# WilliamLewww/lens_trace

Hardware: AMD Instinct MI355X
Metric: Mrays/s (primary+secondary+shadow), 1M-tri @4K (higher is better)
Workload: dtype f32

## Files before the change

### include/lenstrace_hip.h

```cpp
#ifndef LENSTRACE_HIP_H
#define LENSTRACE_HIP_H

#include <stddef.h>
#include <stdint.h>

#ifdef __cplusplus
extern "C" {
#endif

#define LT_HIP_ABI_VERSION 4

typedef struct lt_hip_context lt_hip_context;

enum {
  LT_OK = 0,
  LT_ERR_INVALID_ARGUMENT = 1,
  LT_ERR_NO_DEVICE = 2,
  LT_ERR_HIP = 3,
  LT_ERR_NO_SCENE = 4,
  LT_ERR_BAD_SCENE = 5,
  LT_ERR_BUFFER_TOO_SMALL = 6,
  LT_ERR_UNKNOWN_PROGRAM = 7
};

// ... 301 lines not shown

int lt_hip_entry_cut_chunk_counts(lt_hip_context* ctx, uint64_t* out23);

int lt_hip_read_entry_cuts(lt_hip_context* ctx, void* out, uint64_t capacity, uint64_t* out_bytes);

int lt_hip_entry_cut_pruned_test_host(const uint32_t* refs, const uint16_t* parents, const uint16_t* kids, const uint8_t* survives, uint32_t n,
                                      uint32_t cap, uint32_t* out, uint32_t* count);

int lt_hip_entry_cut_chunks_test_host(const int32_t* heights, const uint32_t* chunks, const uint32_t* entries, const uint32_t* which, uint64_t n,
                                      uint32_t* out);

int lt_hip_entry_cut_triangle_test_host(const float* origins, const float* light_boxes, const float* triangles, uint64_t n, uint8_t* out);

int lt_hip_clear_item_counts(lt_hip_context* ctx, uint64_t* out5);

int lt_hip_clear_items_test_host(const uint32_t* marks, const uint32_t* order, uint32_t n, uint32_t groups, uint32_t tile_w, uint32_t tile_h,
                                 uint32_t tiles_in_call, uint32_t* table, uint8_t* map);

#ifdef __cplusplus
}
#endif
#endif
```

### lens_trace_amd/_capi.py

```python
import ctypes
import os

_HERE = os.path.dirname(os.path.abspath(__file__))
LIB_PATH = os.environ.get("LT_HIP_LIBRARY") or os.path.join(_HERE, "lib", "liblenstrace-hip.so")

(LT_OK, LT_ERR_INVALID_ARGUMENT, LT_ERR_NO_DEVICE, LT_ERR_HIP, LT_ERR_NO_SCENE, LT_ERR_BAD_SCENE,
 LT_ERR_BUFFER_TOO_SMALL, LT_ERR_UNKNOWN_PROGRAM) = range(8)
STATUS_NAMES = ["LT_OK", "LT_ERR_INVALID_ARGUMENT", "LT_ERR_NO_DEVICE", "LT_ERR_HIP", "LT_ERR_NO_SCENE",
                "LT_ERR_BAD_SCENE", "LT_ERR_BUFFER_TOO_SMALL", "LT_ERR_UNKNOWN_PROGRAM"]

PROGRAM_BASIC, PROGRAM_BASIC_LIGHTING, PROGRAM_ACCUMULATOR, PROGRAM_GLOBAL_ILLUMINATION, PROGRAM_GLOBAL_ILLUMINATION_25 = range(5)
PROGRAM_CUSTOM_OPENCL = 5
KERNEL_MODE_LINEAR, KERNEL_MODE_TILE = 0, 1
RENDER_FLAG_STATS = 1
RENDER_FLAG_PIXEL_COUNTERS = 2
RENDER_FLAG_DEVICE_LIBM = 4
RENDER_FLAG_PORTABLE_MATH = 8
RENDER_FLAG_STRICT_MATH = 16
RENDER_FLAG_NO_WALK_TIMING = 32
TRACE_CLOSEST, TRACE_ANY = 0, 1
TRACE_FLAG_COHERENT = 0x100
TRACE_FIRST_K, TRACE_COUNT = 0, 1
TRACE_MAX_HITS = 8
TRACE_LIST_FLAG_FILL_ONLY = 0x200
# ... 11 lines not shown
           "lt_hip_synchronize", "lt_hip_get_stats", "lt_hip_own_hierarchy", "lt_hip_own_wide", "lt_hip_read_scene_structure",
           "lt_hip_trace_rays", "lt_hip_trace_rays_device", "lt_hip_trace_hits", "lt_hip_trace_hits_device",
           "lt_hip_trace_hits_list", "lt_hip_trace_hits_list_device",
           "lt_hip_shade_rays", "lt_hip_shade_rays_device", "lt_hip_shade_paths", "lt_hip_shade_paths_device",
           "lt_hip_trace_surface", "lt_hip_trace_surface_device", "lt_hip_surface_at", "lt_hip_surface_at_device",
           "lt_hip_nearest_points", "lt_hip_nearest_points_device", "lt_hip_nearest_points_host",
           "lt_hip_nearest_k", "lt_hip_nearest_k_device", "lt_hip_nearest_k_host",
           "lt_hip_nearest_list", "lt_hip_nearest_list_device", "lt_hip_nearest_list_host",
           "lt_hip_overlap_boxes", "lt_hip_overlap_boxes_device", "lt_hip_overlap_boxes_host",
           "lt_hip_overlap_tris", "lt_hip_overlap_tris_device", "lt_hip_overlap_tris_host",
           "lt_hip_overlap_boxes_list", "lt_hip_overlap_boxes_list_device", "lt_hip_overlap_boxes_list_host",
           "lt_hip_overlap_tris_list", "lt_hip_overlap_tris_list_device", "lt_hip_overlap_tris_list_host",
           "lt_hip_entry_cut_counts", "lt_hip_entry_cut_test_host",
           "lt_hip_entry_cut_leaf_counts", "lt_hip_entry_cut_triangle_test_host",
           "lt_hip_entry_cut_chunk_counts", "lt_hip_entry_cut_chunks_test_host", "lt_hip_read_entry_cuts",
           "lt_hip_entry_cut_pruned_test_host", "lt_hip_clear_item_counts", "lt_hip_clear_items_test_host"]


class RenderDesc(ctypes.Structure):
    _fields_ = [("struct_size", ctypes.c_uint32), ("program", ctypes.c_int32), ("kernel_mode", ctypes.c_int32),
                ("width", ctypes.c_uint32), ("height", ctypes.c_uint32), ("depth", ctypes.c_uint32),
                ("camera", ctypes.c_uint8 * 28),
                ("frame_first", ctypes.c_uint32), ("frame_count", ctypes.c_uint32), ("accumulate", ctypes.c_uint32),
                ("accumulate_base", ctypes.c_uint32),
                ("tile_w", ctypes.c_uint32), ("tile_h", ctypes.c_uint32), ("tile_first", ctypes.c_uint32),
                ("tile_stride", ctypes.c_uint32),
                ("gi_max_depth", ctypes.c_int32), ("flags", ctypes.c_uint32)]


class Stats(ctypes.Structure):
    _fields_ = [("rays", ctypes.c_uint64), ("shadow_rays", ctypes.c_uint64), ("node_visits", ctypes.c_uint64),
# ... 244 lines not shown
        L.lt_hip_entry_cut_chunk_counts.argtypes = [vp, ctypes.POINTER(u64)]
        L.lt_hip_entry_cut_chunk_counts.restype = i32
        L.lt_hip_entry_cut_chunks_test_host.argtypes = [vp, vp, vp, vp, u64, vp]
        L.lt_hip_entry_cut_chunks_test_host.restype = i32
    if hasattr(L, "lt_hip_read_entry_cuts"):
        L.lt_hip_read_entry_cuts.argtypes = [vp, vp, u64, ctypes.POINTER(u64)]
        L.lt_hip_read_entry_cuts.restype = i32
    if hasattr(L, "lt_hip_entry_cut_pruned_test_host"):
        L.lt_hip_entry_cut_pruned_test_host.argtypes = [vp, vp, vp, vp, ctypes.c_uint32, ctypes.c_uint32, vp, vp]
        L.lt_hip_entry_cut_pruned_test_host.restype = i32
    if hasattr(L, "lt_hip_clear_item_counts"):
        L.lt_hip_clear_item_counts.argtypes = [vp, ctypes.POINTER(u64)]
        L.lt_hip_clear_item_counts.restype = i32
        L.lt_hip_clear_items_test_host.argtypes = [vp, vp] + [ctypes.c_uint32] * 5 + [vp, vp]
        L.lt_hip_clear_items_test_host.restype = i32
    for name in EXPORTS:
        if not hasattr(L, name) and os.environ.get("LT_HIP_LIBRARY"):
            continue
        if name not in ("lt_hip_last_error",):
            getattr(L, name).restype = i32
    if L.lt_hip_abi_version() != 4:
        raise ImportError("liblenstrace-hip.so ABI version mismatch")
    _lib = L
    return L


def program_from_path(path):
    out = ctypes.c_int(0)
    rc = load().lt_hip_program_from_path(path.encode(), ctypes.byref(out))
    if rc:
# ... 36 lines not shown
```

### lens_trace_amd/csrc/lt_capi.hip

```cpp
#include "lt_kernel.hpp"
#include "lt_retree.hpp"
#include "lt_own16.hpp"
#include "lt_prep.hpp"
#include "lt_query.hpp"
#include "lt_nearest.hpp"
#include "lt_overlap.hpp"
#include "lt_tritri.hpp"
#include "lt_overlist.hpp"
#include "lt_shade.hpp"
#include "lt_paths.hpp"

#include "../../include/lenstrace_hip.h"

#include <dlfcn.h>

#include <sched.h>

#include <algorithm>
#include <atomic>
#include <chrono>
#include <exception>
#include <thread>
#include <type_traits>
#include <cmath>
// ... 311 lines not shown
  bool cuts_valid = false;
  unsigned long long* d_cut_stats = nullptr;
  uint32_t cuts_leaves = 0;
  uint32_t cuts_chunks = 0;
  uint32_t cuts_node_chunks = 0;
  uint32_t cuts_plane_squares = 0;
  uint64_t cut_builds = 0;
  uint32_t* d_items = nullptr;
  uint64_t items_words = 0;
  uint32_t* d_foldmap = nullptr;
  uint64_t foldmap_words = 0;
  uint32_t items_groups = 0;
  bool items_folds = false;
  unsigned long long* d_item_stats = nullptr;
  uint64_t item_builds = 0;
  bool last_folded = false;
  bool last_tabled = false;
  unsigned long long* h_item_stats = nullptr;
  hipEvent_t items_ev = nullptr;
  int items_worth = -1;
  uint64_t scene_generation = 0;
  hipEvent_t render_ev = nullptr;
  hipStream_t render_stream = nullptr;
  bool render_ev_recorded = false;
  uint64_t d_samples_bytes = 0;
  uint32_t* d_order = nullptr;
  uint64_t order_capacity = 0;
  std::vector<uint32_t> order_key;
  uint32_t order_head[8] = {0};
  int cu_count = 256;
// ... 726 lines not shown
  bool fused_frames = !env_off("LT_FUSED_FRAMES");
  uint64_t fused_bytes = 16ull << 30;
  uint32_t debug_lds_rows = 0;
  bool debug_calibration = getenv("LT_DEBUG_CALIBRATION") != nullptr;
  bool debug_camera_hits = getenv("LT_DEBUG_CAMERA_HITS") != nullptr;
  bool pinned_readback = !env_off("LT_PINNED_READBACK");
  bool camera_hits = !env_off("LT_CAMERA_HITS");
  bool camera_hits_keep = !env_off("LT_CAMERA_HITS_KEEP");
  bool entry_cut = !env_off("LT_ENTRY_CUT");
  uint32_t entry_cut_leaves = 512;
  uint32_t entry_cut_chunks = (uint32_t)lt_entry_cut::kDefaultChunks;
  uint32_t entry_cut_node_chunks = (uint32_t)lt_entry_cut::kDefaultNodeChunks;
  bool clear_items = !env_off("LT_CLEAR_ITEMS");
  bool clear_items_fold = true;
  bool clear_items_force = false;
  uint32_t shadow_frames = 2;
  bool debug_shadow_frames = getenv("LT_DEBUG_SHADOW_FRAMES") != nullptr;
  RenderKnobs() {
    if (const char* e = getenv("LT_SHADOW_PACKETS")) shadow_packets = std::max(0, std::min(3, atoi(e)));
    if (const char* e = getenv("LT_SHADOW_SPREAD")) shadow_spread = (float)atof(e);
    if (const char* e = getenv("LT_GI_MEGAKERNEL")) gi_wavefront = atoi(e) == 0;
    if (const char* e = getenv("LT_TRACE_REFILL")) trace_refill = (uint32_t)std::max(1, std::min(64, atoi(e)));
    if (const char* e = getenv("LT_FUSED_BYTES")) fused_bytes = strtoull(e, nullptr, 10);
    if (const char* e = getenv("LT_DEBUG_LDS_ROWS")) debug_lds_rows = (uint32_t)std::max(1, std::min(160, atoi(e)));
    if (const char* e = getenv("LT_ENTRY_CUT_LEAVES")) {
      const int v = atoi(e);
      entry_cut_leaves = v <= 0 ? 0u : v == 1 ? 512u : (uint32_t)std::min(v, 1 << 20);
    }
    if (const char* e = getenv("LT_ENTRY_CUT_CHUNKS")) entry_cut_chunks = (uint32_t)std::max(1, std::min(lt_entry_cut::kMaxChunks, atoi(e)));
    if (const char* e = getenv("LT_ENTRY_CUT_NODE_CHUNKS")) entry_cut_node_chunks = (uint32_t)std::max(1, std::min(lt_entry_cut::kMaxChunks, atoi(e)));
// ... 670 lines not shown
                            hipStream_t s, const RenderKnobs& k, ReadBack* rb) {
  if (const int rc = check_render_desc(ctx, d, p, out_device, out_bytes)) return rc;
  LT_HIP_CHECK(ctx, hipSetDevice(ctx->device));
  const bool stats = (d->flags & (LT_RENDER_FLAG_STATS | LT_RENDER_FLAG_PIXEL_COUNTERS)) != 0;
  const int devlibm = (d->flags & LT_RENDER_FLAG_PORTABLE_MATH) ? 0 : (d->flags & LT_RENDER_FLAG_STRICT_MATH) ? 1 : 2;
  SceneDev sc = scene_dev(ctx, k, devlibm);
  FrameParams fp = frame_params(d, p, k);
  uint32_t camFrame;
  memcpy(&camFrame, d->camera + 24, 4);
  const uint32_t frames = d->frame_count ? d->frame_count : 1;
  const uint64_t nblocks = p.squares();

  if (!ctx->render_ev) LT_HIP_CHECK(ctx, hipEventCreateWithFlags(&ctx->render_ev, hipEventDisableTiming));
  if (ctx->render_ev_recorded && s != ctx->render_stream) LT_HIP_CHECK(ctx, hipStreamWaitEvent(s, ctx->render_ev, 0));
  if (stats) LT_HIP_CHECK(ctx, hipMemsetAsync(ctx->d_stats, 0, 8 * sizeof(unsigned long long), s));
  if (k.persistent) {
    const uint64_t queueBytes = ((uint64_t)frames + 1) * 8 * kQueueStride * sizeof(uint32_t);
    LT_HIP_CHECK(ctx, grow_scratch(ctx, ctx->d_queues, ctx->queue_frames, (uint64_t)frames + 1, queueBytes));
    LT_HIP_CHECK(ctx, hipMemsetAsync(ctx->d_queues, 0, queueBytes, s));
    if (k.square_order)
      if (const int rc = ensure_square_order(ctx, d, p, fp.sinYaw == 0.0f, s, &fp.order, fp.orderHead)) return rc;
  }
  FusionPlan fu;
  if (const int rc = plan_fusion(ctx, k, d, p, frames, stats, fp.giMaxDepth, fu)) return rc;
  const bool fused = fu.chunk > 1, meanInLaunch = d->frame_count && d->accumulate && !fused;
  const uint32_t firstFrames = fused ? std::min(fu.chunk, frames) : 1u;
  const std::vector<uint32_t> shadowKey = {(uint32_t)d->program, d->width, d->height, p.tileW, p.tileH, p.tileFirst, p.tileStride,
                                           firstFrames == 1u ? 1u : firstFrames < 8u ? 2u : 8u};
  const bool queueOk = d->program == LT_PROGRAM_ACCUMULATOR && k.persistent && !stats && ctx->d_rank8 != nullptr && !meanInLaunch &&
                       nblocks * firstFrames * kBlock + (uint64_t)ctx->cu_count * 2048u <= 0xffffffffull;
// ... 40 lines not shown
      float* outPtr = out;
      void* args[] = {(void*)&sc, (void*)&fp, (void*)&outPtr, (void*)&statsPtr, (void*)&queues};
      const hipFunction_t fn = devlibm == 2 ? up.lds : devlibm == 1 ? up.ldsStrict : up.ldsPortable;
      LT_HIP_CHECK(ctx, hipModuleLaunchKernel(fn, grid.x, 1, 1, kBlock, 1, 1, lds, s, args, nullptr));
    } else {
      FrameParams fl = fp;
      const uint32_t groups = (nf + 1u) / 2u;
      if (k.clear_items && k.persistent && !stats && d->program == LT_PROGRAM_ACCUMULATOR && (shadowMode == 1 || shadowMode == 2) && fp.entryCuts != nullptr && ctx->cuts_valid && fp.cameraHits != nullptr &&
          std::all_of(fp.orderHead, fp.orderHead + 8, [](uint32_t h) { return h == 0u; }) && std::min(shadowGroup, k.shadow_frames) >= 2u &&
          nf >= 2u && fp.squareMajor != 0u && nblocks * groups < 0x80000000ull) {
        const bool fold = k.clear_items_fold && fused && mean_in_quads(fp.depth, paddedTiles, out_device) && p.tileW % 8u == 0u;
        if (const int rc = ensure_clear_items(ctx, call, fl, groups, fold, p.floats, out_device, (int32_t)(d->accumulate_base + f))) return rc;
      }
      foldMap = (const unsigned char*)fl.foldMap;
      tabled = fl.itemTable != nullptr;
      if (shadowMode < 0 && calibrate)
        if (const int rc = calibrate_shadow_walk(ctx, call, sc, fp, grid, out, queues, queueOk, shadowKey, shadowMode, shadowGroup)) return rc;
      if (const int rc = launch_walk(ctx, call, sc, (uint32_t)std::max(0, shadowMode), shadowGroup, fl, grid, out, queues)) return rc;
    }
    LT_HIP_CHECK(ctx, hipGetLastError());
    call.launches++;
    if (fp.storeHeadHits) {
      ctx->camhits_key.swap(hitsKey);
      fp.storeHeadHits = 0u;
    }
    if (fused)
      if (const int rc = launch_running_mean(ctx, s, fp, p.floats, nf, (int32_t)(d->accumulate_base + f), paddedTiles, out_device, f + nf >= frames ? rb : nullptr, foldMap))
        return rc;
    ctx->last_folded = (launchIndex != 0 && ctx->last_folded) || foldMap != nullptr;
    ctx->last_tabled = (launchIndex != 0 && ctx->last_tabled) || tabled;
// ... 1524 lines not shown
  out4[0] = out4[1] = out4[2] = 0;
  out5[4] = ctx->last_tabled ? 1 : 0;
  out4[3] = ctx->item_builds;
  if (ctx->cuts_valid && ctx->items_groups != 0u && ctx->d_item_stats) {
    LT_HIP_CHECK(ctx, hipSetDevice(ctx->device));
    if (ctx->render_ev_recorded) LT_HIP_CHECK(ctx, hipEventSynchronize(ctx->render_ev));
    unsigned long long h[2];
    LT_HIP_CHECK(ctx, hipMemcpy(h, ctx->d_item_stats, sizeof(h), hipMemcpyDeviceToHost));
    out4[0] = h[0];
    out4[1] = h[1];
    out4[2] = ctx->last_folded ? h[1] : 0;
  }
  return LT_OK;
}

extern "C" int lt_hip_clear_items_test_host(const uint32_t* marks, const uint32_t* order, uint32_t n, uint32_t groups, uint32_t tile_w, uint32_t tile_h,
                                            uint32_t tiles_in_call, uint32_t* table, uint8_t* map) {
  if (!marks || !table || groups == 0 || (uint64_t)n * groups >= 0x80000000ull) return LT_ERR_INVALID_ARGUMENT;
  const uint32_t bptx = (tile_w + 7u) / 8u, bpty = (tile_h + 7u) / 8u;
  if (map && (tile_w == 0 || tile_w % 8u != 0 || tile_h == 0 || (uint64_t)tiles_in_call * bptx * bpty != n)) return LT_ERR_INVALID_ARGUMENT;
  for (uint32_t xcd = 0; xcd < 8u; xcd++) {
    const uint32_t share = xcd_share_size(n, xcd), start = xcd_share_start(n, xcd);
    uint32_t* const dst = table + lt_entry_cut::kItemHeader + (size_t)start * groups;
    uint32_t at = 0;
    for (uint32_t local = 0; local < share; local++) {
      const uint32_t word0 = marks[start + local];
      lt_entry_cut::item_write(dst + at, word0, local, groups);
      at += lt_entry_cut::item_entries(word0, groups);
      if (map) {
        const uint32_t b = order ? order[start + local] : start + local;
// ... 36 lines not shown
```

### lens_trace_amd/csrc/lt_device.hpp

```cpp
#pragma once
#ifndef __HIPCC_RTC__
#include <hip/hip_runtime.h>
#include <stdint.h>
#else
typedef unsigned char uint8_t;
typedef unsigned short uint16_t;
typedef unsigned int uint32_t;
typedef int int32_t;
typedef unsigned long long uint64_t;
#endif

#ifndef M_PI
#define M_PI 3.14159265358979323846
#endif

#include "lt_walk_asm.hpp"

namespace lt {

constexpr int kBlock = 64;
constexpr int kLdsStack = 32;
constexpr int kQueueStride = 64;
constexpr int kPacketEntry = 4;
constexpr int kPacketRows = 2;
constexpr int kMaxStack = 64;
constexpr int kOwnRows = 16;
constexpr int kOwnDeep = 48;
constexpr int kTraceRows = 10;
constexpr int kTraceStage = 10;
constexpr float kFltMax = 3.402823466e+38f;
constexpr uint32_t kDeadSlot = 0xffffffffu;

enum Program { kBasic = 0, kBasicLighting = 1, kAccumulator = 2, kGI = 3, kGI25 = 4, kCustom = 5,
               kAccumulatorQueue = 7,
               kGIPrimary = 6,
               kUser = 1000 };

// ... 886 lines not shown
        traverse_own_lane<PROGRAM, ANYHIT>(sc, ray, ix, iy, iz, useIgnore ? ignore : -1, pl, st.lds);
        return;
      }
    }
  }
  if constexpr (STATS || LDSSCENE) {
    if (__all(finite)) traverse_nodes_impl<PROGRAM, Stack<DEEP>, STATS, true, ANYHIT, LDSSCENE>(sc, ray, ix, iy, iz, useIgnore, ignore, pl, st, c);
    else traverse_nodes_impl<PROGRAM, Stack<DEEP>, STATS, false, ANYHIT, LDSSCENE>(sc, ray, ix, iy, iz, useIgnore, ignore, pl, st, c);
  } else {
    ScratchStack ss;
    traverse_nodes_impl<PROGRAM, ScratchStack, false, false, ANYHIT, false>(sc, ray, ix, iy, iz, useIgnore, ignore, pl, ss, c);
  }
}

constexpr uint32_t kEntryCutClear = 0xffffffffu;
template <int PROGRAM, class CFG>
__device__ inline bool traverse_shadow2(const SceneDev& sc, const Ray (&ray)[2], int ignore, Hit (&pl)[2], Stack<CFG::kDeep>& st, Counters& c,
                                        const uint32_t* cut, uint32_t cutPlane, uint32_t cutChunks) {
  bool ok = false;
  if constexpr (!CFG::kStats && !CFG::kDeep && !CFG::kLdsScene) {
    float inv[2][3];
    ok = sc.shadowPackets == 1u || sc.shadowPackets == 2u;
    unsigned long long sign[2][3];
    const unsigned long long all = __builtin_amdgcn_ballot_w64(true);
#pragma unroll
    for (int j = 0; j < 2; j++) {
      inv[j][0] = 1.0f / ray[j].d.x; inv[j][1] = 1.0f / ray[j].d.y; inv[j][2] = 1.0f / ray[j].d.z;
      const bool finite = __builtin_fabsf(inv[j][0]) < __builtin_inff() && __builtin_fabsf(inv[j][1]) < __builtin_inff() &&
                          __builtin_fabsf(inv[j][2]) < __builtin_inff() && __builtin_fabsf(ray[j].o.x) < __builtin_inff() &&
                          __builtin_fabsf(ray[j].o.y) < __builtin_inff() && __builtin_fabsf(ray[j].o.z) < __builtin_inff();
      ok = ok && __all(finite) && sc.rank8 != nullptr && __all(packet_ray_ok(ray[j], inv[j][0], inv[j][1], inv[j][2]));
      if (ok && sc.shadowPackets == 2u) {
        auto first = [](float v) { return __int_as_float(__builtin_amdgcn_readfirstlane(__float_as_int(v))); };
        const float rx = first(ray[j].o.x), ry = first(ray[j].o.y), rz = first(ray[j].o.z);
        const float ex = ray[j].o.x - rx, ey = ray[j].o.y - ry, ez = ray[j].o.z - rz;
        ok = __builtin_amdgcn_ballot_w64(ex * ex + ey * ey + ez * ez > sc.shadowSpread * (pl[j].t * pl[j].t)) == 0ull;
      }
#pragma unroll
      for (int a = 0; a < 3; a++) sign[j][a] = __builtin_amdgcn_ballot_w64(inv[j][a] < 0.0f);
    }
    uint32_t neg = 0u, mixed = 0u;
#pragma unroll
    for (int a = 0; a < 3; a++) {
      neg |= sign[0][a] != 0ull ? 1u << a : 0u;
      mixed |= (sign[0][a] == 0ull || sign[0][a] == all) && sign[1][a] == sign[0][a] ? 0u : 1u << a;
    }
    ok = ok && (mixed & (mixed - 1u)) == 0u;
    uint32_t form = neg;
    if (mixed == 1u) form = 8u + (neg >> 1);
    else if (mixed == 2u) form = 12u + ((neg & 1u) | (neg >> 1 & 2u));
    else if (mixed == 4u) form = 16u + (neg & 3u);
    if (sc.groupWalks != nullptr && (int)__lane_id() == __ffsll((long long)all) - 1) {
      atomicAdd(&sc.groupWalks[ok ? 0 : 1], 1ull);
      if (ok && form >= 8u) atomicAdd(&sc.groupWalks[form - 6u], 1ull);
    }
    if (ok && cut != nullptr && *(const __attribute__((address_space(4))) uint32_t*)(unsigned long long)cut == kEntryCutClear) return true;
    if (ok) {
      int* const row = st.lds - __lane_id();
      switch (form) {
        case 0: packet_walk2<PROGRAM, 0>(sc, ray, inv, ignore, pl, row, cut, cutPlane, cutChunks); break;
        case 1: packet_walk2<PROGRAM, 1>(sc, ray, inv, ignore, pl, row, cut, cutPlane, cutChunks); break;
        case 2: packet_walk2<PROGRAM, 2>(sc, ray, inv, ignore, pl, row, cut, cutPlane, cutChunks); break;
        case 3: packet_walk2<PROGRAM, 3>(sc, ray, inv, ignore, pl, row, cut, cutPlane, cutChunks); break;
        case 4: packet_walk2<PROGRAM, 4>(sc, ray, inv, ignore, pl, row, cut, cutPlane, cutChunks); break;
        case 5: packet_walk2<PROGRAM, 5>(sc, ray, inv, ignore, pl, row, cut, cutPlane, cutChunks); break;
        case 6: packet_walk2<PROGRAM, 6>(sc, ray, inv, ignore, pl, row, cut, cutPlane, cutChunks); break;
// ... 366 lines not shown
  unsigned long long frameStride;
  const uint32_t* order;
  uint32_t orderHead[8];
  uint4* cameraHits;
  uint32_t shadowFrames;
  uint32_t storeHeadHits;
  const uint32_t* entryCuts;
  uint32_t entryCutPlane;
  uint32_t entryCutChunks;
  const uint32_t* itemTable;
  const uint32_t* foldMap;
  float* foldOut;
  int32_t foldBase;
  uint32_t itemGroups;
};

__host__ __device__ inline float running_mean_step(float acc, float c, int32_t n) {
  if (n <= 0) return c;
  const float nf = (float)n, n1 = (float)(n + 1);
  return (c + (acc * nf)) / n1;
}

template <int DEVLIBM>
__device__ __forceinline__ Ray camera_ray(const FrameParams& fp, int x, int y, float& fx, float& fy) {
  const V4 cameraPosition = mk4(fp.camx, fp.camy, fp.camz, 1.0f);
  const V4 film = mk4(Math<DEVLIBM>::fdiv((float)x, (float)fp.width) - 0.5f, Math<DEVLIBM>::fdiv((float)y, (float)fp.height) - 0.5f, 0.0f, 1.0f);
  const V4 aperture = mk4(fp.apx, fp.apy, fp.apz, 1.0f);
  Ray ray{add4(cameraPosition, film), sub4(aperture, film)};
  const float cy = DEVLIBM ? ::cosf(fp.yaw) : fp.cosYaw, sy = DEVLIBM ? ::sinf(fp.yaw) : fp.sinYaw;
  const float newX = Math<DEVLIBM>::mad(cy, ray.d.x, sy * ray.d.z);
// ... 72 lines not shown
```

### lens_trace_amd/csrc/lt_kernel.hpp

```cpp
#pragma once
#include "lt_device.hpp"
#include "lt_entry_cut.hpp"

using namespace lt;

__device__ __forceinline__ uint32_t xcd_remap(uint32_t b, uint32_t n) {
  const uint32_t q = n / 8u, r = n % 8u, xcd = b % 8u;
  return (xcd < r ? xcd * (q + 1u) : r * (q + 1u) + (xcd - r) * q) + b / 8u;
}

__host__ __device__ inline uint32_t xcd_share_size(uint32_t n, uint32_t xcd) { return n / 8u + (xcd < n % 8u ? 1u : 0u); }
__host__ __device__ inline uint32_t xcd_share_start(uint32_t n, uint32_t xcd) {
  const uint32_t q = n / 8u, r = n % 8u;
  return xcd < r ? xcd * (q + 1u) : r * (q + 1u) + (xcd - r) * q;
}
constexpr uint32_t kClaimPair = 2u;
__host__ __device__ inline uint32_t camera_hit_squares(const FrameParams& fp, uint32_t xcd) {
  return xcd_share_size(fp.totalSquares, xcd) - (fp.order ? fp.orderHead[xcd] : 0u);
}

__device__ __forceinline__ bool square_pixel(const FrameParams& fp, uint32_t b, uint32_t& x, uint32_t& y, uint32_t& pix) {
  const uint32_t k = b / fp.blocksPerTile, sb = b % fp.blocksPerTile;
  const uint32_t sbx = sb % fp.blocksPerTileX, sby = sb / fp.blocksPerTileX;
  const uint32_t tile = fp.tileFirst + k * fp.tileStride;
// ... 66 lines not shown
      } else {
        store(frame, color);
      }
    }
    if (STATS) {
      c.rays += pc.rays; c.shadow += pc.shadow; c.nodes += pc.nodes; c.tris += pc.tris;
#ifdef LT_DEBUG_WAVE_COUNTERS
      c.wInner += pc.wInner; c.wTri += pc.wTri; c.wOuter += pc.wOuter;
#endif
    }
  }
  if (queueing && !queued) ((uint4*)sc.shadowQueue)[2 * (size_t)sc.shadowCap + qslot] = make_uint4(kDeadSlot, 0u, 0u, 0u);
}

template <class CFG>
__device__ __forceinline__ void camera_hit_square(const SceneDev& sc, const FrameParams& fp, uint32_t b, uint32_t pos, Stack<CFG::kDeep>& st, Counters& c) {
  uint32_t x, y, pix;
  Hit pl{0, 0, kFltMax, 0.0f, 0.0f};
  if (square_pixel(fp, b, x, y, pix)) {
    float fx, fy;
    const Ray ray = camera_ray<CFG::kDevLibm>(fp, (int)x, (int)y, fx, fy);
    pl = camera_hit<kAccumulator, CFG>(sc, ray, nullptr, st, c);
  }
  fp.cameraHits[(size_t)pos * kBlock + threadIdx.x] = make_uint4((uint32_t)pl.prim, (uint32_t)pl.hitType, __float_as_uint(pl.u), __float_as_uint(pl.v));
}

#ifndef LT_GI_WAVES
#define LT_GI_WAVES 5
#endif
#ifndef LT_GI_STAGE_WAVES
// ... 6 lines not shown

template <int PROGRAM, class CFG, bool HITS = false>
__device__ __forceinline__ void render_kernel_body(const SceneDev& sc, const FrameParams& fp, float* __restrict__ out,
                                                   unsigned long long* __restrict__ stats, uint32_t* __restrict__ queues) {
  extern __shared__ int lds_stack[];
  constexpr bool STATS = CFG::kStats;
  Stack<CFG::kDeep> st;
  st.lds = lds_stack + threadIdx.x;
  st.rows = (int)fp.ldsRows;
  Counters c{};

  const uint32_t home = fp.persistent ? (__builtin_amdgcn_s_getreg((3u << 11) | 20u) & 7u) : 0u;
  uint32_t sweep = 0;
  uint32_t claimed = 0, claimedLeft = 0;
  uint32_t wholeNext = 0u;
  uint32_t tableLimit = 0u, tableSweep = 8u;
  auto sload = [](const uint32_t* p) { return *(const __attribute__((address_space(4))) uint32_t*)(unsigned long long)p; };
  bool done = false;
  while (!done) {
    uint32_t b, frame = 0, frames = 1, pos = 0;
    bool stored = false;
    bool folding = false;
    if (!fp.persistent) {
      b = xcd_remap(blockIdx.x, gridDim.x);
      pos = b;
      done = true;
    } else {
      const uint32_t xcd = (home + sweep) & 7u;
      const uint32_t share = xcd_share_size(fp.totalSquares, xcd), start = xcd_share_start(fp.totalSquares, xcd);
      const uint32_t head = fp.order ? fp.orderHead[xcd] : 0u;
      const uint32_t group = PROGRAM == kAccumulator && CFG::kGroups && !STATS && !HITS && fp.cameraHits != nullptr && fp.shadowFrames >= 2u ? 2u : 1u;
      const uint32_t groups = (fp.fusedFrames + group - 1u) / group;
      const bool table = PROGRAM == kAccumulator && CFG::kGroups && CFG::kItems && !STATS && !HITS && group == 2u && fp.itemTable != nullptr &&
                         fp.itemGroups == groups && fp.squareMajor != 0u && head == 0u;
      if (table && tableSweep != sweep) {
        tableLimit = sload(fp.itemTable + xcd);
        tableSweep = sweep;
      }
      const uint32_t limit = table ? tableLimit : HITS ? camera_hit_squares(fp, xcd) : head * fp.fusedFrames + (share - head) * groups;
      uint32_t t = 0;
      if (table && wholeNext != 0u) {
        folding = (wholeNext & lt_entry_cut::kItemWhole) != 0u;
        t = wholeNext & ~lt_entry_cut::kItemWhole;
        wholeNext = (t + 1u) % groups == 0u ? 0u : wholeNext + 1u;
      } else {
        if (claimedLeft == 0u) {
          const uint32_t take = limit / 4u > gridDim.x && (!table || limit / share > groups / 2u) ? kClaimPair : 1u;
          if (threadIdx.x == 0) t = atomicAdd(&queues[xcd * kQueueStride], take);
          claimed = (uint32_t)__builtin_amdgcn_readfirstlane((int)t);
// ... 4 lines not shown
        if (t >= limit) {
          claimedLeft = 0u;
          done = ++sweep >= 8u;
          continue;
        }
        if (table) {
          const uint32_t entry = sload(fp.itemTable + lt_entry_cut::kItemHeader + (size_t)start * groups + t);
          t = entry & ~lt_entry_cut::kItemWhole;
          if ((entry & lt_entry_cut::kItemWhole) != 0u) {
            if (fp.foldMap != nullptr) {
              const uint32_t sq = fp.order ? sload(fp.order + start + t / groups) : start + t / groups;
              const uint32_t k = sq / fp.blocksPerTile, sb = sq % fp.blocksPerTile;
              const unsigned long long seg = lt_entry_cut::fold_segment(k, fp.tileH, fp.tileW, sb / fp.blocksPerTileX * 8u, sb % fp.blocksPerTileX);
              folding = (sload(fp.foldMap + (seg >> 2)) >> (8u * (uint32_t)(seg & 3ull)) & 0xffu) != 0u;
            }
            wholeNext = groups == 1u ? 0u : (t + 1u) | (folding ? lt_entry_cut::kItemWhole : 0u);
          }
        }
      }
      stored = fp.cameraHits != nullptr && t >= head * fp.fusedFrames;
      if (HITS) {
        t += head;
      } else if (t < head * fp.fusedFrames) {
        frame = t / head;
        t -= frame * head;
      } else if (fp.fusedFrames > 1u) {
        t -= head * fp.fusedFrames;
        uint32_t item;
        if (fp.squareMajor) {
          item = t % groups;
          t = head + t / groups;
// ... 1 lines not shown
          item = t / (share - head);
          t = head + (t - item * (share - head));
        }
        frame = item * group;
        frames = fp.fusedFrames - frame < group ? fp.fusedFrames - frame : group;
      }
      b = start + t;
      pos = b;
      if (fp.order) b = (uint32_t)__builtin_amdgcn_readfirstlane((int)fp.order[b]);
    }
    if (HITS) {
      camera_hit_square<CFG>(sc, fp, b, pos, st, c);
    } else {
      render_square<PROGRAM, CFG>(sc, fp, out, b, frame, frames, st, c, pos, stored ? fp.cameraHits + (size_t)pos * kBlock : nullptr,
                                  stored && fp.entryCuts != nullptr ? fp.entryCuts + (size_t)pos * lt_entry_cut::kListWords : nullptr, folding);
    }
  }
  if (STATS) {
    atomicAdd(&stats[0], (unsigned long long)c.rays);
    atomicAdd(&stats[1], (unsigned long long)c.shadow);
    atomicAdd(&stats[2], (unsigned long long)c.nodes);
    atomicAdd(&stats[3], (unsigned long long)c.tris);
#ifdef LT_DEBUG_WAVE_COUNTERS
    atomicAdd(&stats[4], (unsigned long long)c.wInner);
    atomicAdd(&stats[5], (unsigned long long)c.wTri);
    atomicAdd(&stats[6], (unsigned long long)c.wOuter);
#endif
  }
}

// ... 678 lines not shown
```

### lens_trace_amd/renderer.py

```python
import ctypes
from dataclasses import dataclass, field
from typing import Optional

import numpy as np

from . import _capi as C
from .scene import Scene

KERNEL_MODE_LINEAR, KERNEL_MODE_TILE = C.KERNEL_MODE_LINEAR, C.KERNEL_MODE_TILE
THREAD_ORGANIZATION_MODE_MAX_FIT, THREAD_ORGANIZATION_MODE_CUSTOM = 0, 1


@dataclass
class ThreadOrganizationHIP:
    blockSize: tuple = (0, 0)


@dataclass
class RenderPropertiesHIP:
    kernelFilePath: str
    imageDimensions: tuple
    pOutputBuffer: np.ndarray
    pAccelerationStructureExplicit: Scene
    pModel: Optional[Scene] = None
# ... 408 lines not shown
                "plain": (int(out[5]), int(out[6])), "squares_by_chunks": {k: int(out[6 + k]) for k in range(1, 17)}}

    def entry_cuts(self):
        n = ctypes.c_uint64(0)
        self._check(self._L.lt_hip_read_entry_cuts(self._ctx, None, ctypes.c_uint64(0), ctypes.byref(n)))
        if n.value == 0:
            return None
        buf = np.zeros(n.value // 4, dtype=np.uint32)
        self._check(self._L.lt_hip_read_entry_cuts(self._ctx, buf.ctypes.data_as(ctypes.c_void_p), ctypes.c_uint64(buf.nbytes), ctypes.byref(n)))
        return buf.reshape(-1, 16)

    def clear_item_counts(self):
        out = (ctypes.c_uint64 * 5)()
        self._check(self._L.lt_hip_clear_item_counts(self._ctx, out))
        return {"entries": int(out[0]), "whole": int(out[1]), "folded": int(out[2]), "builds": int(out[3]), "used": bool(out[4])}

    def scene_structure(self, what):
        from . import scene as sc
        n = ctypes.c_uint64(0)
        self._check(self._L.lt_hip_read_scene_structure(self._ctx, what, None, ctypes.c_uint64(0), ctypes.byref(n)))
        if n.value == 0:
            return None
        buf = np.zeros(n.value, dtype=np.uint8)
        self._check(self._L.lt_hip_read_scene_structure(self._ctx, what, buf.ctypes.data_as(ctypes.c_void_p), ctypes.c_uint64(buf.nbytes), ctypes.byref(n)))
        if what == 0:
            return buf.view(sc.NODE_DTYPE)
        if what == 1:
            return buf.view(np.uint32).reshape(-1, 8)
        if what == 3:
            return tuple(int(x) for x in buf.view(np.int32))
# ... 183 lines not shown
```

Baseline: 65660.

## Render clear squares in one pass across all frame groups without shadow walks

Adds a one-pass path for squares whose entry cut marks them clear: it loops over all fused frame groups inside one item, computing direct lighting from stored camera hits, and skips the shadow traversal as long as the wave still qualifies for a joint walk and every light is listed. The packet-eligibility test is moved into a shared helper so this path can reuse it. Squares that stop qualifying hand the remaining groups back to the normal per-group item path. The aim is to cut per-item scheduling and repeated hit and setup loads. In exchange it adds complexity, per-square counters written with atomics into spare queue slots, and a new C API to read those counters.

```diff
diff --git a/include/lenstrace_hip.h b/include/lenstrace_hip.h
--- a/include/lenstrace_hip.h
+++ b/include/lenstrace_hip.h
@@ -339,6 +339,8 @@
 
 int lt_hip_clear_item_counts(lt_hip_context* ctx, uint64_t* out5);
 
+int lt_hip_clear_square_counts(lt_hip_context* ctx, uint64_t* out3);
+
 int lt_hip_clear_items_test_host(const uint32_t* marks, const uint32_t* order, uint32_t n, uint32_t groups, uint32_t tile_w, uint32_t tile_h,
                                  uint32_t tiles_in_call, uint32_t* table, uint8_t* map);
 
diff --git a/lens_trace_amd/_capi.py b/lens_trace_amd/_capi.py
--- a/lens_trace_amd/_capi.py
+++ b/lens_trace_amd/_capi.py
@@ -49,7 +49,8 @@
            "lt_hip_entry_cut_counts", "lt_hip_entry_cut_test_host",
            "lt_hip_entry_cut_leaf_counts", "lt_hip_entry_cut_triangle_test_host",
            "lt_hip_entry_cut_chunk_counts", "lt_hip_entry_cut_chunks_test_host", "lt_hip_read_entry_cuts",
-           "lt_hip_entry_cut_pruned_test_host", "lt_hip_clear_item_counts", "lt_hip_clear_items_test_host"]
+           "lt_hip_entry_cut_pruned_test_host", "lt_hip_clear_item_counts", "lt_hip_clear_items_test_host",
+           "lt_hip_clear_square_counts"]
 
 
 class RenderDesc(ctypes.Structure):
@@ -324,6 +325,9 @@
         L.lt_hip_clear_item_counts.restype = i32
         L.lt_hip_clear_items_test_host.argtypes = [vp, vp] + [ctypes.c_uint32] * 5 + [vp, vp]
         L.lt_hip_clear_items_test_host.restype = i32
+    if hasattr(L, "lt_hip_clear_square_counts"):
+        L.lt_hip_clear_square_counts.argtypes = [vp, ctypes.POINTER(u64)]
+        L.lt_hip_clear_square_counts.restype = i32
     for name in EXPORTS:
         if not hasattr(L, name) and os.environ.get("LT_HIP_LIBRARY"):
             continue
diff --git a/lens_trace_amd/csrc/lt_capi.hip b/lens_trace_amd/csrc/lt_capi.hip
--- a/lens_trace_amd/csrc/lt_capi.hip
+++ b/lens_trace_amd/csrc/lt_capi.hip
@@ -349,6 +349,7 @@
   bool items_folds = false;
   unsigned long long* d_item_stats = nullptr;
   uint64_t item_builds = 0;
+  const uint32_t* last_clear_queues = nullptr;
   bool last_folded = false;
   bool last_tabled = false;
   unsigned long long* h_item_stats = nullptr;
@@ -1105,6 +1106,7 @@
   bool clear_items = !env_off("LT_CLEAR_ITEMS");
   bool clear_items_fold = true;
   bool clear_items_force = false;
+  bool clear_square = !env_off("LT_CLEAR_SQUARE");
   uint32_t shadow_frames = 2;
   bool debug_shadow_frames = getenv("LT_DEBUG_SHADOW_FRAMES") != nullptr;
   RenderKnobs() {
@@ -1805,6 +1807,7 @@
   if (!ctx->render_ev) LT_HIP_CHECK(ctx, hipEventCreateWithFlags(&ctx->render_ev, hipEventDisableTiming));
   if (ctx->render_ev_recorded && s != ctx->render_stream) LT_HIP_CHECK(ctx, hipStreamWaitEvent(s, ctx->render_ev, 0));
   if (stats) LT_HIP_CHECK(ctx, hipMemsetAsync(ctx->d_stats, 0, 8 * sizeof(unsigned long long), s));
+  ctx->last_clear_queues = nullptr;
   if (k.persistent) {
     const uint64_t queueBytes = ((uint64_t)frames + 1) * 8 * kQueueStride * sizeof(uint32_t);
     LT_HIP_CHECK(ctx, grow_scratch(ctx, ctx->d_queues, ctx->queue_frames, (uint64_t)frames + 1, queueBytes));
@@ -1875,6 +1878,9 @@
       }
       foldMap = (const unsigned char*)fl.foldMap;
       tabled = fl.itemTable != nullptr;
+      const bool onePass = tabled && k.clear_square && !k.debug_shadow_frames;
+      if (onePass) fl.itemGroups |= kItemGroupsOnePass;
+      ctx->last_clear_queues = onePass ? queues : nullptr;
       if (shadowMode < 0 && calibrate)
         if (const int rc = calibrate_shadow_walk(ctx, call, sc, fp, grid, out, queues, queueOk, shadowKey, shadowMode, shadowGroup)) return rc;
       if (const int rc = launch_walk(ctx, call, sc, (uint32_t)std::max(0, shadowMode), shadowGroup, fl, grid, out, queues)) return rc;
@@ -3429,6 +3435,23 @@
   return LT_OK;
 }
 
+extern "C" int lt_hip_clear_square_counts(lt_hip_context* ctx, uint64_t* out3) {
+  if (!ctx || !out3) return LT_ERR_INVALID_ARGUMENT;
+  out3[0] = out3[1] = out3[2] = 0;
+  if (ctx->last_clear_queues == nullptr) return LT_OK;
+  LT_HIP_CHECK(ctx, hipSetDevice(ctx->device));
+  if (ctx->render_ev_recorded) LT_HIP_CHECK(ctx, hipEventSynchronize(ctx->render_ev));
+  uint32_t h[8 * kQueueStride];
+  LT_HIP_CHECK(ctx, hipMemcpy(h, ctx->last_clear_queues, sizeof(h), hipMemcpyDeviceToHost));
+  for (uint32_t xcd = 0; xcd < 8u; xcd++)
+    for (uint32_t i = 0; i < 3u; i++) {
+      uint64_t v;
+      memcpy(&v, h + xcd * kQueueStride + kClearCountAt + 2u * i, sizeof(v));
+      out3[i] += v;
+    }
+  return LT_OK;
+}
+
 extern "C" int lt_hip_clear_items_test_host(const uint32_t* marks, const uint32_t* order, uint32_t n, uint32_t groups, uint32_t tile_w, uint32_t tile_h,
                                             uint32_t tiles_in_call, uint32_t* table, uint8_t* map) {
   if (!marks || !table || groups == 0 || (uint64_t)n * groups >= 0x80000000ull) return LT_ERR_INVALID_ARGUMENT;
diff --git a/lens_trace_amd/csrc/lt_device.hpp b/lens_trace_amd/csrc/lt_device.hpp
--- a/lens_trace_amd/csrc/lt_device.hpp
+++ b/lens_trace_amd/csrc/lt_device.hpp
@@ -21,6 +21,7 @@
 constexpr int kBlock = 64;
 constexpr int kLdsStack = 32;
 constexpr int kQueueStride = 64;
+constexpr int kClearCountAt = 32;
 constexpr int kPacketEntry = 4;
 constexpr int kPacketRows = 2;
 constexpr int kMaxStack = 64;
@@ -937,42 +938,52 @@
 }
 
 constexpr uint32_t kEntryCutClear = 0xffffffffu;
+
+__device__ __forceinline__ bool shadow_frames_walk_together(const SceneDev& sc, const Ray (&ray)[2], const float (&tmax)[2], unsigned long long& all,
+                                                            float (&inv)[2][3], uint32_t& form) {
+  bool ok = sc.shadowPackets == 1u || sc.shadowPackets == 2u;
+  unsigned long long sign[2][3];
+  all = __builtin_amdgcn_ballot_w64(true);
+#pragma unroll
+  for (int j = 0; j < 2; j++) {
+    inv[j][0] = 1.0f / ray[j].d.x; inv[j][1] = 1.0f / ray[j].d.y; inv[j][2] = 1.0f / ray[j].d.z;
+    const bool finite = __builtin_fabsf(inv[j][0]) < __builtin_inff() && __builtin_fabsf(inv[j][1]) < __builtin_inff() &&
+                        __builtin_fabsf(inv[j][2]) < __builtin_inff() && __builtin_fabsf(ray[j].o.x) < __builtin_inff() &&
+                        __builtin_fabsf(ray[j].o.y) < __builtin_inff() && __builtin_fabsf(ray[j].o.z) < __builtin_inff();
+    ok = ok && __all(finite) && sc.rank8 != nullptr && __all(packet_ray_ok(ray[j], inv[j][0], inv[j][1], inv[j][2]));
+    if (ok && sc.shadowPackets == 2u) {
+      auto first = [](float v) { return __int_as_float(__builtin_amdgcn_readfirstlane(__float_as_int(v))); };
+      const float rx = first(ray[j].o.x), ry = first(ray[j].o.y), rz = first(ray[j].o.z);
+      const float ex = ray[j].o.x - rx, ey = ray[j].o.y - ry, ez = ray[j].o.z - rz;
+      ok = __builtin_amdgcn_ballot_w64(ex * ex + ey * ey + ez * ez > sc.shadowSpread * (tmax[j] * tmax[j])) == 0ull;
+    }
+#pragma unroll
+    for (int a = 0; a < 3; a++) sign[j][a] = __builtin_amdgcn_ballot_w64(inv[j][a] < 0.0f);
+  }
+  uint32_t neg = 0u, mixed = 0u;
+#pragma unroll
+  for (int a = 0; a < 3; a++) {
+    neg |= sign[0][a] != 0ull ? 1u << a : 0u;
+    mixed |= (sign[0][a] == 0ull || sign[0][a] == all) && sign[1][a] == sign[0][a] ? 0u : 1u << a;
+  }
+  ok = ok && (mixed & (mixed - 1u)) == 0u;
+  form = neg;
+  if (mixed == 1u) form = 8u + (neg >> 1);
+  else if (mixed == 2u) form = 12u + ((neg & 1u) | (neg >> 1 & 2u));
+  else if (mixed == 4u) form = 16u + (neg & 3u);
+  return ok;
+}
+
 template <int PROGRAM, class CFG>
 __device__ inline bool traverse_shadow2(const SceneDev& sc, const Ray (&ray)[2], int ignore, Hit (&pl)[2], Stack<CFG::kDeep>& st, Counters& c,
                                         const uint32_t* cut, uint32_t cutPlane, uint32_t cutChunks) {
   bool ok = false;
   if constexpr (!CFG::kStats && !CFG::kDeep && !CFG::kLdsScene) {
     float inv[2][3];
-    ok = sc.shadowPackets == 1u || sc.shadowPackets == 2u;
-    unsigned long long sign[2][3];
-    const unsigned long long all = __builtin_amdgcn_ballot_w64(true);
-#pragma unroll
-    for (int j = 0; j < 2; j++) {
-      inv[j][0] = 1.0f / ray[j].d.x; inv[j][1] = 1.0f / ray[j].d.y; inv[j][2] = 1.0f / ray[j].d.z;
-      const bool finite = __builtin_fabsf(inv[j][0]) < __builtin_inff() && __builtin_fabsf(inv[j][1]) < __builtin_inff() &&
-                          __builtin_fabsf(inv[j][2]) < __builtin_inff() && __builtin_fabsf(ray[j].o.x) < __builtin_inff() &&
-                          __builtin_fabsf(ray[j].o.y) < __builtin_inff() && __builtin_fabsf(ray[j].o.z) < __builtin_inff();
-      ok = ok && __all(finite) && sc.rank8 != nullptr && __all(packet_ray_ok(ray[j], inv[j][0], inv[j][1], inv[j][2]));
-      if (ok && sc.shadowPackets == 2u) {
-        auto first = [](float v) { return __int_as_float(__builtin_amdgcn_readfirstlane(__float_as_int(v))); };
-        const float rx = first(ray[j].o.x), ry = first(ray[j].o.y), rz = first(ray[j].o.z);
-        const float ex = ray[j].o.x - rx, ey = ray[j].o.y - ry, ez = ray[j].o.z - rz;
-        ok = __builtin_amdgcn_ballot_w64(ex * ex + ey * ey + ez * ez > sc.shadowSpread * (pl[j].t * pl[j].t)) == 0ull;
-      }
-#pragma unroll
-      for (int a = 0; a < 3; a++) sign[j][a] = __builtin_amdgcn_ballot_w64(inv[j][a] < 0.0f);
-    }
-    uint32_t neg = 0u, mixed = 0u;
-#pragma unroll
-    for (int a = 0; a < 3; a++) {
-      neg |= sign[0][a] != 0ull ? 1u << a : 0u;
-      mixed |= (sign[0][a] == 0ull || sign[0][a] == all) && sign[1][a] == sign[0][a] ? 0u : 1u << a;
-    }
-    ok = ok && (mixed & (mixed - 1u)) == 0u;
-    uint32_t form = neg;
-    if (mixed == 1u) form = 8u + (neg >> 1);
-    else if (mixed == 2u) form = 12u + ((neg & 1u) | (neg >> 1 & 2u));
-    else if (mixed == 4u) form = 16u + (neg & 3u);
+    unsigned long long all;
+    const float tmax[2] = {pl[0].t, pl[1].t};
+    uint32_t form;
+    ok = shadow_frames_walk_together(sc, ray, tmax, all, inv, form);
     if (sc.groupWalks != nullptr && (int)__lane_id() == __ffsll((long long)all) - 1) {
       atomicAdd(&sc.groupWalks[ok ? 0 : 1], 1ull);
       if (ok && form >= 8u) atomicAdd(&sc.groupWalks[form - 6u], 1ull);
@@ -1369,6 +1380,9 @@
   int32_t foldBase;
   uint32_t itemGroups;
 };
+constexpr uint32_t kItemGroupsOnePass = 0x80000000u;
+__host__ __device__ inline uint32_t item_groups(const FrameParams& fp) { return fp.itemGroups & ~kItemGroupsOnePass; }
+__host__ __device__ inline bool item_one_pass(const FrameParams& fp) { return (fp.itemGroups & kItemGroupsOnePass) != 0u; }
 
 __host__ __device__ inline float running_mean_step(float acc, float c, int32_t n) {
   if (n <= 0) return c;
diff --git a/lens_trace_amd/csrc/lt_kernel.hpp b/lens_trace_amd/csrc/lt_kernel.hpp
--- a/lens_trace_amd/csrc/lt_kernel.hpp
+++ b/lens_trace_amd/csrc/lt_kernel.hpp
@@ -104,6 +104,143 @@
 }
 
 template <class CFG>
+__device__ __forceinline__ uint32_t render_clear_square(const SceneDev& sc, const FrameParams& fp, float* __restrict__ out, uint32_t b, uint32_t pos,
+                                                        uint32_t groups, bool fold, uint32_t (&count)[3]) {
+  if (*(const __attribute__((address_space(4))) uint32_t*)(unsigned long long)(fp.entryCuts + (size_t)pos * lt_entry_cut::kListWords) != kEntryCutClear) return 0u;
+  count[0]++;
+  const uint32_t k = b / fp.blocksPerTile, sb = b % fp.blocksPerTile;
+  const uint32_t sbx = sb % fp.blocksPerTileX, sby = sb / fp.blocksPerTileX;
+  const uint32_t tile = fp.tileFirst + k * fp.tileStride;
+  const uint32_t tx = tile % fp.tilesX, ty = tile / fp.tilesX;
+  const uint32_t lane = threadIdx.x;
+  const uint32_t lx = sbx * 8u + (lane & 7u);
+  const uint32_t ly = sby * 8u + (lane >> 3);
+  const uint32_t x = tx * fp.tileW + lx, y = ty * fp.tileH + ly;
+  const bool valid = k < fp.tilesInCall && lx < fp.tileW && ly < fp.tileH && x < fp.width && y < fp.height;
+  const size_t first = (((size_t)k * fp.tileH + ly) * fp.tileW + lx) * fp.depth;
+  bool shaded = false;
+  float flat = 0.0f;
+  float fx = 0.0f, fy = 0.0f;
+  V4 position = mk4(0.0f, 0.0f, 0.0f, 1.0f), normal = mk4(0.0f, 0.0f, 0.0f, 0.0f);
+  V3 diffuse{0.0f, 0.0f, 0.0f};
+  if (valid) {
+    (void)camera_ray<CFG::kDevLibm>(fp, (int)x, (int)y, fx, fy);
+    const uint4 h = (fp.cameraHits + (size_t)pos * kBlock)[__lane_id()];
+    const int prim = (int)h.x;
+    if (is_light(sc.lights, prim)) flat = 1.0f;
+    else shaded = (int)h.y == 1;
+    if (shaded) {
+      const float* pr = prim_ptr(sc, prim);
+      const V3 bc = barycentrics(__uint_as_float(h.z), __uint_as_float(h.w));
+      const V3 p3 = bary3<CFG::kDevLibm>(pr + 0, pr + 3, pr + 6, bc);
+      position = mk4(p3.x, p3.y, p3.z, 1.0f);
+      const V3 n3 = bary3<CFG::kDevLibm>(pr + 9, pr + 12, pr + 15, bc);
+      normal = mk4(n3.x, n3.y, n3.z, 0.0f);
+      const Material* m = sc.mats + prim_material(pr);
+      diffuse = V3{m->diffuse[0], m->diffuse[1], m->diffuse[2]};
+    }
+  }
+  const bool anyShaded = __builtin_amdgcn_ballot_w64(shaded) != 0ull;
+  float mean[3] = {0.0f, 0.0f, 0.0f};
+  if (fold && valid) {
+    const float* d = fp.foldOut + first;
+    mean[0] = d[0]; mean[1] = d[1]; mean[2] = d[2];
+  }
+  auto store = [&](uint32_t f, const V3& color) {
+    if (fold) {
+      const int32_t n = fp.foldBase + (int32_t)f;
+      mean[0] = running_mean_step(mean[0], color.x, n);
+      mean[1] = running_mean_step(mean[1], color.y, n);
+      mean[2] = running_mean_step(mean[2], color.z, n);
+    } else {
+      float* d = out + (size_t)f * fp.frameStride + first;
+      const int32_t n = fp.accumulateN;
+      if (n <= 0) {
+        d[0] = color.x; d[1] = color.y; d[2] = color.z;
+      } else {
+        d[0] = running_mean_step(d[0], color.x, n);
+        d[1] = running_mean_step(d[1], color.y, n);
+        d[2] = running_mean_step(d[2], color.z, n);
+      }
+    }
+  };
+  const uint32_t full = fp.fusedFrames / 2u;
+  float carried[2] = {0.0f, 0.0f};
+  uint32_t g = 0u;
+#pragma unroll 1
+  for (uint32_t it = 0u; it <= full; it++) {
+    bool together = false;
+    float ndotl[2] = {0.0f, 0.0f};
+    if (shaded) {
+      float rnd[4];
+      rnd[0] = carried[0];
+      rnd[1] = carried[1];
+      uint32_t opaque = sc.shadowPackets;
+      asm volatile("" : "+s"(opaque));
+      const uint32_t s = fp.frameCount + 2u * it;
+      if (opaque == 0xffffffffu) {
+#pragma unroll
+        for (int i = 0; i < 2; i++) rnd[2 + i] = __uint_as_float(opaque + (uint32_t)i);
+      } else {
+#pragma unroll
+        for (int i = 0; i < 2; i++) rnd[2 + i] = random_<CFG::kDevLibm>(fx, fy, (float)(s + (uint32_t)i));
+      }
+      carried[0] = rnd[2];
+      carried[1] = rnd[3];
+      if (it != 0u) {
+        V4 lightPosition[2];
+        bool listed = true;
+#pragma unroll
+        for (int j = 0; j < 2; j++) {
+          const float* lp = light_prim(sc, rnd[j]);
+          listed = listed && light_index_listed(sc, rnd[j]);
+          float uvx = rnd[j + 1], uvy = rnd[j + 2];
+          if (uvx + uvy > 1.0f) {
+            uvx = 1.0f - uvx;
+            uvy = 1.0f - uvy;
+          }
+          const V3 l3 = bary3<CFG::kDevLibm>(lp + 0, lp + 3, lp + 6, barycentrics(uvx, uvy));
+          lightPosition[j] = mk4(l3.x, l3.y, l3.z, 1.0f);
+        }
+        asm volatile("" ::: "memory");
+        Ray ray[2];
+        float tmax[2];
+#pragma unroll
+        for (int j = 0; j < 2; j++) {
+          const V4 toLight = normalize4<CFG::kDevLibm>(sub4(lightPosition[j], position));
+          tmax[j] = (float)((double)distance4<CFG::kDevLibm>(position, lightPosition[j]) - 0.01);
+          ndotl[j] = dot4(toLight, normal);
+          ray[j] = Ray{position, toLight};
+        }
+        asm volatile("" : "+v"(ndotl[0]), "+v"(ndotl[1]));
+        float inv[2][3];
+        uint32_t form;
+        unsigned long long all;
+        together = shadow_frames_walk_together(sc, ray, tmax, all, inv, form) && __builtin_amdgcn_ballot_w64(!listed) == 0ull;
+      }
+    }
+    if (it == 0u) continue;
+    if (anyShaded && __builtin_amdgcn_ballot_w64(together) == 0ull) break;
+    if (valid) {
+#pragma unroll
+      for (int j = 0; j < 2; j++) {
+        V3 color = shaded ? V3{diffuse.x * ndotl[j], diffuse.y * ndotl[j], diffuse.z * ndotl[j]} : V3{flat, flat, flat};
+        if (fp.clampOutput) color = V3{Math<CFG::kDevLibm>::clamp01(color.x), Math<CFG::kDevLibm>::clamp01(color.y), Math<CFG::kDevLibm>::clamp01(color.z)};
+        store(2u * (it - 1u) + (uint32_t)j, color);
+      }
+    }
+    g = it;
+    count[2]++;
+  }
+  if (fold && valid && g != 0u) {
+    float* d = fp.foldOut + first;
+    d[0] = mean[0]; d[1] = mean[1]; d[2] = mean[2];
+  }
+  if (g != groups) count[1]++;
+  return g;
+}
+
+template <class CFG>
 __device__ __forceinline__ void camera_hit_square(const SceneDev& sc, const FrameParams& fp, uint32_t b, uint32_t pos, Stack<CFG::kDeep>& st, Counters& c) {
   uint32_t x, y, pix;
   Hit pl{0, 0, kFltMax, 0.0f, 0.0f};
@@ -140,6 +277,8 @@
   uint32_t sweep = 0;
   uint32_t claimed = 0, claimedLeft = 0;
   uint32_t wholeNext = 0u;
+  constexpr bool kClearSquare = PROGRAM == kAccumulator && CFG::kGroups && CFG::kItems && !STATS && !HITS;
+  uint32_t clearCount[3] = {0u, 0u, 0u};
   uint32_t tableLimit = 0u, tableSweep = 8u;
   auto sload = [](const uint32_t* p) { return *(const __attribute__((address_space(4))) uint32_t*)(unsigned long long)p; };
   bool done = false;
@@ -158,7 +297,7 @@
       const uint32_t group = PROGRAM == kAccumulator && CFG::kGroups && !STATS && !HITS && fp.cameraHits != nullptr && fp.shadowFrames >= 2u ? 2u : 1u;
       const uint32_t groups = (fp.fusedFrames + group - 1u) / group;
       const bool table = PROGRAM == kAccumulator && CFG::kGroups && CFG::kItems && !STATS && !HITS && group == 2u && fp.itemTable != nullptr &&
-                         fp.itemGroups == groups && fp.squareMajor != 0u && head == 0u;
+                         item_groups(fp) == groups && fp.squareMajor != 0u && head == 0u;
       if (table && tableSweep != sweep) {
         tableLimit = sload(fp.itemTable + xcd);
         tableSweep = sweep;
@@ -193,7 +332,15 @@
               const unsigned long long seg = lt_entry_cut::fold_segment(k, fp.tileH, fp.tileW, sb / fp.blocksPerTileX * 8u, sb % fp.blocksPerTileX);
               folding = (sload(fp.foldMap + (seg >> 2)) >> (8u * (uint32_t)(seg & 3ull)) & 0xffu) != 0u;
             }
-            wholeNext = groups == 1u ? 0u : (t + 1u) | (folding ? lt_entry_cut::kItemWhole : 0u);
+            if constexpr (kClearSquare) {
+              if (item_one_pass(fp) && sc.groupWalks == nullptr && fp.entryCuts != nullptr) {
+                const uint32_t at = start + t / groups;
+                const uint32_t rendered = render_clear_square<CFG>(sc, fp, out, fp.order ? sload(fp.order + at) : at, at, groups, folding, clearCount);
+                if (rendered == groups) continue;
+                t += rendered;
+              }
+            }
+            wholeNext = (t + 1u) % groups == 0u ? 0u : (t + 1u) | (folding ? lt_entry_cut::kItemWhole : 0u);
           }
         }
       }
@@ -225,6 +372,13 @@
     } else {
       render_square<PROGRAM, CFG>(sc, fp, out, b, frame, frames, st, c, pos, stored ? fp.cameraHits + (size_t)pos * kBlock : nullptr,
                                   stored && fp.entryCuts != nullptr ? fp.entryCuts + (size_t)pos * lt_entry_cut::kListWords : nullptr, folding);
+    }
+  }
+  if constexpr (kClearSquare) {
+    if (clearCount[0] != 0u && threadIdx.x == 0u) {
+      unsigned long long* const at = (unsigned long long*)(queues + home * kQueueStride + kClearCountAt);
+#pragma unroll
+      for (int i = 0; i < 3; i++) atomicAdd(&at[i], (unsigned long long)clearCount[i]);
     }
   }
   if (STATS) {
diff --git a/lens_trace_amd/renderer.py b/lens_trace_amd/renderer.py
--- a/lens_trace_amd/renderer.py
+++ b/lens_trace_amd/renderer.py
@@ -446,6 +446,11 @@
         out = (ctypes.c_uint64 * 5)()
         self._check(self._L.lt_hip_clear_item_counts(self._ctx, out))
         return {"entries": int(out[0]), "whole": int(out[1]), "folded": int(out[2]), "builds": int(out[3]), "used": bool(out[4])}
+
+    def clear_square_counts(self):
+        out = (ctypes.c_uint64 * 3)()
+        self._check(self._L.lt_hip_clear_square_counts(self._ctx, out))
+        return {"entered": int(out[0]), "left": int(out[1]), "groups": int(out[2])}
 
     def scene_structure(self, what):
         from . import scene as sc
```

New measurement: 73890 (median of 6 runs). +12.5%, better.
